# metatensor/metatrain

Hardware: AMD Instinct MI355X
Metric: atom-steps/sec (energy+forces) PET 10k-atom box (higher is better)
Workload: dtype f32; 1 GPU; PET forward + dE/dR (preprocess+features+predict+backward), 8 x 10000-atom boxes per GPU per step, default PET hypers (2.9M params), 4.5 A cutoff, 191050 edges/box; parallelism=boxes sharded over 1 rank(s), no data-path collective

## Files before the change

### metatrain_amd/csrc/model.h

```cpp
#pragma once
#include <map>
#include <set>
#include <string>
#include <vector>

#include "common.h"
#include "switches.h"

namespace pet {

constexpr int D = 128;
constexpr int DN = 256;
constexpr int DFF = 256;
constexpr int DNF = 2 * DN;
constexpr int DH = 128;
constexpr int NHEAD = 8;
constexpr int HD = D / NHEAD;
constexpr int MAX_SPECIES = 128;

struct Lin {
    const float* w = nullptr;
    const float* b = nullptr;
    float4* fwd = nullptr;
    float4* bwd = nullptr;
// ... 140 lines not shown
constexpr int MAILBOX_INTS = 64;
int read_back(const int* d_a, int na, const int* d_b, int nb, int* out, hipStream_t st);
int64_t graph_workspace_bytes(int64_t n_nodes, int64_t e0);
int graph_attention_lists(const Graph& g, hipStream_t st);
int graph_build(const Model& m, const float* pos, const float* cells, const int* centers,
                const int* neighbors, const int* shifts, const int* species, const int* sys,
                int64_t n_nodes, int64_t e0, int64_t n_systems, void* ws, int64_t ws_bytes,
                Graph& g, hipStream_t st);
int graph_check_reverse(Graph& g, hipStream_t st);
int64_t graph_from_batch_workspace_bytes(int64_t n_nodes, int64_t max_nbr);
int graph_from_batch(const int64_t* el_nodes, const int64_t* el_nbr, const float* ev, const float* ed, const uint8_t* mask,
                     const int64_t* rni, const float* cf, int64_t n_nodes, int64_t max_nbr, void* ws, int64_t ws_bytes,
                     Graph& g, hipStream_t st);
int graph_export(const Graph& g, float cutoff, int64_t* el_nodes, int64_t* el_nbr, float* ev,
                 float* ed, uint8_t* mask, int64_t* rni, float* cf, float* stats, int64_t* centers,
                 int64_t* neighbors, int64_t* slot, int64_t* shifts, hipStream_t st);
int sum_over_atoms(const Graph& g, const float* atomic, float* out, hipStream_t st);

int64_t nl_workspace_bytes(int64_t n_atoms);
int64_t nl_batch_workspace_bytes(int64_t n_atoms, int64_t n_systems);
int nl_build_batch(const float* d_pos, const float* h_cells, const int* h_pbc, const int64_t* h_first_atom, int64_t n_sys,
                   float cutoff, void* ws, int* d_pairs, float* d_vectors, int64_t capacity, int64_t* n_pairs,
                   hipStream_t st);
int nl_build(const float* d_pos, const float* h_cell, const int* h_pbc, int64_t n, float cutoff,
             void* ws, int* d_pairs, float* d_vectors, int64_t capacity, int64_t* n_pairs,
             hipStream_t st);

bool use_generic(const Model& m, const Graph& g);

int64_t gen_workspace_bytes(const Model& m, int64_t n_nodes, int64_t n_edges);
int gen_forward_layers(const Model& m, const Graph& g, void* ws, int64_t ws_bytes, int save, float* atomic,
                       float* const* node_feats, float* const* edge_feats, int n_layers, hipStream_t st);
int gen_backward_features(const Model& m, const Graph& g, void* ws, int64_t ws_bytes, const float* const* g_node,
                          const float* const* g_edge, int n_layers, float* g_geo, float* g_fc, hipStream_t st);
int gen_backward(const Model& m, const Graph& g, void* ws, int64_t ws_bytes, const float* gA, float* gpos, float* gcell,
                 hipStream_t st);
int gen_predict(const Model& m, const Graph& g, const HeadW& H, const LastW& Lw, const float* node_feat,
                const float* edge_feat, const float* fc, float* atomic, float* node_hidden, float* edge_hidden,
                hipStream_t st);
int gen_predict_backward(const Model& m, const Graph& g, const HeadW& H, const LastW& Lw, const float* node_feat,
                         const float* edge_feat, const float* fc, const float* gA, float* g_node, float* g_edge, float* g_fc,
                         hipStream_t st);
int gen_aux_outputs(const Model& m, const Graph& g, const float* node_feat, const float* edge_feat, float* feature,
                    float* last_layer, float* scratch, hipStream_t st);
int gen_backward_predict(const Model& m, const Graph& g, void* ws, int64_t ws_bytes, const float* gA, float* g_node,
                         float* g_edge, float* g_fc, hipStream_t st);
int gen_backward_geometry(const Model& m, const Graph& g, void* ws, int64_t ws_bytes, const float* g_geo, const float* g_fc,
                          float* gpos, float* gcell, hipStream_t st);
int64_t gen_train_workspace_bytes(const Model& m, int64_t n_nodes, int64_t n_edges);
int norm_rev_rows(const float* Xp, const float* Xt, const float* gamma, int ln, float eps, const float* NYp, const float* NYt,
                  float* NXp, float* NXt, int64_t R, int W, hipStream_t st);
struct HvpTaps {
    float *ngeo, *lgeo;
    float *sb, *sdb;
    float *db, *dbd;
    float *dfc, *dfcd;
    float* dv;
};
int gen_train2(const Model& m, const Graph& g, void* ws2, int64_t ws2_bytes, const float* lA, const float* nA, const float* u,
               const float* ucell, float* tangent_atomic, hipStream_t st, const float* const* seed_node = nullptr,
               const float* const* seed_edge = nullptr, int n_seed = 0, const HvpTaps* hv = nullptr);
int64_t gen_hvp_workspace_bytes(const Model& m, int64_t n_nodes, int64_t n_edges);
int gen_hvp(const Model& m, const Graph& g, void* ws, int64_t ws_bytes, const float* lA, const float* u, const float* ucell,
            float* hvp_pos, float* hvp_cell, float* tangent_atomic, hipStream_t st);
int gen_train_predict(const Model& m, const Graph& g, void* ws, int64_t ws_bytes, int layer, const HeadW& H, const LastW& Lw,
                      float* atomic, hipStream_t st);
int gen_train_predict_backward(const Model& m, const Graph& g, void* ws, int64_t ws_bytes, int layer, const HeadW& H,
                               int n_blocks, const LastW* const* Lw, const float* const* gA, float* seed_node,
                               float* seed_edge, hipStream_t st);
inline bool train_generic(const Model& m) { return m.generic() || !m.trainable(); }
inline bool train_generic_for(const Model& m, const Graph& g) { return train_generic(m) || use_generic(m, g) || g.n_edges == 0; }
bool generic_workspace(const Graph& g, const void* ws);
int backward_geometry_generic(const Model& m, const Graph& g, float* dv_scratch, const float* dgeo, const float* dfc_a,
                              const float* dfc_b, float* gpos, float* gcell, hipStream_t st);

int64_t forward_workspace_bytes(const Model& m, int64_t n_nodes, int64_t n_edges, bool train = false);
int forward(const Model& m, const Graph& g, void* ws, int64_t ws_bytes, int save, float* atomic,
            float* node_feat, float* edge_feat, hipStream_t st);
int forward_layers(const Model& m, const Graph& g, void* ws, int64_t ws_bytes, int save, float* atomic,
                   float* const* node_feats, float* const* edge_feats, int n_layers, hipStream_t st);
int backward_features_layers_abi(const Model& m, const Graph& g, void* ws, int64_t ws_bytes, const float* const* g_node,
                                 const float* const* g_edge, int n_layers, float* g_geo, float* g_fc, hipStream_t st);
int backward(const Model& m, const Graph& g, void* ws, int64_t ws_bytes, const float* grad_atomic,
             float* grad_pos, float* grad_cells, hipStream_t st);
int64_t predict_scratch_floats(int64_t n_nodes, int64_t n_edges);
int predict(const Model& m, const Graph& g, const HeadW& H, const LastW& Lw, const float* node_feat, const float* edge_feat,
            const float* fc, float* atomic, float* node_hidden, float* edge_hidden, float* scratch, hipStream_t st);
int predict_backward(const Model& m, const Graph& g, const HeadW& H, const LastW& Lw, const float* node_feat,
                     const float* edge_feat, const float* fc, const float* grad_atomic, float* g_node, float* g_edge,
                     float* g_fc, float* scratch, hipStream_t st);
int aux_outputs(const Model& m, const Graph& g, const float* node_feat, const float* edge_feat, float* feature,
                float* last_layer, float* scratch, hipStream_t st);
int backward_train(const Model& m, const Graph& g, void* ws, int64_t ws_bytes, const float* grad_atomic,
                   float* grad_pos, float* grad_cells, hipStream_t st, const float* const* seed_node = nullptr,
                   const float* const* seed_edge = nullptr, int n_seed = 0);
int train_predict(const Model& m, const Graph& g, void* ws, int64_t ws_bytes, int layer, const HeadW& H, const LastW& Lw,
                  float* atomic, hipStream_t st);
int train_predict_backward(const Model& m, const Graph& g, void* ws, int64_t ws_bytes, const std::string& target, int layer,
                           const HeadW& H, int n_blocks, const char* const* blocks, const LastW* const* Lw,
                           const float* const* gA, float* seed_node, float* seed_edge, hipStream_t st);
int llpr_features(const Model& m, const Graph& g, const char* target, const char* block, const float* const* node_feats,
                  const float* const* edge_feats, int n_layers, float* atomic, float* llf, hipStream_t st);
int llpr_rows(const float* llf, int64_t N, int F, const int* sysidx, int64_t S, const uint8_t* mask, int mean, float* rows,
              hipStream_t st);
int llpr_covariance_accumulate(const float* X, int64_t R, int F, double* C, hipStream_t st);
int llpr_covariance_finalize(double* C, int F, hipStream_t st);
int llpr_variance(const float* X, int64_t R, int F, const float* M, float alpha, float* sigma, hipStream_t st);
int llpr_ensemble(const float* X, int64_t R, int F, const float* W, int K, int P, const float* pred, float* Y, hipStream_t st);
int64_t so_workspace_bytes(const Model& m, int64_t n_nodes, int64_t n_edges);
int geometry_tangent(const Model& m, const Graph& g, const float* u, const float* ucell, float* Tgeo, float* Tfc, float* Tkb,
                     hipStream_t st);
int backward_train2(const Model& m, const Graph& g, void* ws, int64_t ws_bytes, void* ws2, int64_t ws2_bytes,
                    const float* lambda_atomic, const float* nu_atomic, const float* u, float* tangent_atomic,
                    hipStream_t st, const float* u_cell = nullptr, const float* const* seed_node = nullptr,
                    const float* const* seed_edge = nullptr, int n_seed = 0);
int backward_predict_abi(const Model& m, const Graph& g, void* ws, int64_t ws_bytes, const float* grad_atomic,
                         float* g_node, float* g_edge, float* g_fc, hipStream_t st);
int backward_features_abi(const Model& m, const Graph& g, void* ws, int64_t ws_bytes, const float* g_node,
                          const float* g_edge, float* g_geo, float* g_fc, hipStream_t st);
int geometry_backward(const Model& m, const Graph& g, const float* g_geo, const float* g_fc, float* gpos, float* gcell,
                      float* scratch, hipStream_t st);
int backward_geometry_abi(const Model& m, const Graph& g, void* ws, int64_t ws_bytes, const float* g_geo,
                          const float* g_fc, float* grad_pos, float* grad_cells, hipStream_t st);

bool use_trr();
int trr_compress(bool first, const Graph& g, const GnnLayerW& G, const float* Min, float* a0_out, float* Xout, int64_t E,
                 hipStream_t st);
int trr_compress_bwd(bool first, const float* dXe, const float* a0, const GnnLayerW& G, float* dgeo, float* dM, int64_t E,
                     float* t_da0, hipStream_t st);
int trr_head_edge(const Model& m, const float* Xin, const float* fc, float* ypred, float* yout, int64_t E, hipStream_t st);
int trr_head_edge_bwd(const Model& m, const float* Xin, const float* gA, const int* ctr, const float* fc, const float* ypred,
                      float* dfc, float* dXout, int64_t E, float* t_s1, float* t_da2, float* t_da1, float* t_s2y, hipStream_t st);
void trr_qkv(const float* X, const float* gamma, const float* beta, const Lin& qkv, float* QKV, int64_t R, hipStream_t st);
void trr_qkv_bwd(const float* dQKV, const float* X, const float* gamma, bool layer_norm, const Lin& qkv, const float* dX1,
                 float* dXin, int64_t E, int64_t R, hipStream_t st);
void trr_oproj(const float* AO, const float* X, const Lin& out, float* X1, float* OC, int64_t E, int64_t R, hipStream_t st);
void trr_oproj_bwd(const float* dX1, const float* dOC, const Lin& out, float* dAO, int64_t E, int64_t R, hipStream_t st);
void trr_emlp(const float* X1, const float* gamma, const float* beta, const Lin& win, const Lin& wout, float* VG, float* X2,
              int64_t E, hipStream_t st);
void trr_emlp_bwd(const float* dY, const float* X1, const float* VG, const float* gamma, const float* beta, const Lin& win,
                  const Lin& wout, float* dX1, int64_t E, hipStream_t st, float* t_dvg = nullptr, int ldy = 128,
                  const float* dY2 = nullptr, const int* rev2 = nullptr);
int trr_comb(bool first, const float* XF, const Graph& g, const GnnLayerW& G, const float* Min, const float* edge_emb, float* CA,
             float* LNS, float* Mout, int64_t E, hipStream_t st);
int trr_comb_bwd(const float* dM, const float* XF, const Graph& g, const GnnLayerW& G, const float* LNS, const float* CA,
                 float* dcat, int64_t E, float* t_da, hipStream_t st, bool add_dm = false);
int emlp_s(const float* X1, const float* gamma, const float* beta, const Lin& win, const Lin& wout, float* VG, float* X2,
           int64_t E, hipStream_t st);
int emlp_bwd_s(const float* dY, const float* X1, bool ln, const Lin& win_g, const Lin& wout, float* dX1, int64_t E,
               hipStream_t st, int ldy, const float* dY2, const int* rev2);
int head_edge_s(const Model& m, const float* Xin, const float* fc, float* ypred, float* yout, int64_t E, hipStream_t st);
int head_edge_bwd_s(const Model& m, const float* Xin, const float* gA, const int* ctr, const float* fc, const float* ypred,
                    float* dfc, float* dXout, int64_t E, hipStream_t st);
int compress_bwd_s(bool first, const float* dXe, const float* a0, const GnnLayerW& G, float* dgeo, float* dM, int64_t E, hipStream_t st);
int comb_s(bool first, const float* XF, const int* rev, const Lin& c0g, const Lin& c2, const float* Min, const float* edge_emb,
           const int* sp_nbr, float* CA, float* LNS, float* Mout, int64_t E, hipStream_t st);
int comb_bwd_s(const float* dM, const float* XF, const int* rev, const float* LNS, const float* CA, const Lin& c0g, const Lin& c2,
               float* dcat, int64_t E, bool add_dm, hipStream_t st);
int center_s(const Lin& cc, const float* H, float* Xc, int64_t N, hipStream_t st);
int expand_bwd_s(const Lin& ce, const float* dH1, float* dOC, int64_t N, hipStream_t st);
int center_bwd_s(const Lin& cc, const float* dC, const float* dH1, float* dHin, int64_t N, hipStream_t st);
int node_fwd_s(const AttnLayerW& A, const float* H, const float* OC, float* H1, float* VGn, float* Hn, float* tmp, int64_t N,
               hipStream_t st);
int node_bwd_s(const AttnLayerW& A, const float* dHn, const float* H1, const float* VGn, float* dH1, float* tmp, int64_t N, bool ln,
               hipStream_t st);
int ablk_fwd(const Model& m, const Graph& g, const AttnLayerW& A, const float* X, float* X1, float* OC, float scale, hipStream_t st);
int ablk_bwd(const Model& m, const Graph& g, const AttnLayerW& A, const float* X, const float* dX1, const float* dOC, float* dXin,
             float* dbias, float scale, hipStream_t st);
void ablk_prof_dump();
bool rowgemm_s(hipStream_t st, const float* X, int K, const float* cs, const void* planes, const float* bias, float* Y, int n_out,
               int64_t R, bool acc);
bool rowgemm_s_ex(hipStream_t st, const float* X, int K, const float* cs, const void* planes, const float* bias, const float* A,
                  float* Y, int n_out, int64_t R, int norm, const float* cb);
bool rowgemm_s_swiglu_bwd(hipStream_t st, const float* X, const void* planes, const float* VG, float* dVG, int hid, int64_t R);
bool rowgemm_s_norm_bwd(hipStream_t st, const float* X, int K, const void* planes, const float* xn, const float* gamma, int ln,
                        const float* dres, float* out, int64_t R);

bool attn_fwd_preload(int nt, const float* QKV, const Graph& g, float* AO, float scale, hipStream_t st);
bool attn_bwd_preload(int nt, const float* QKV, const float* dAO, const Graph& g, float* dQKV, float* dbias_h,
                      float scale, hipStream_t st);

bool attn_jvp_mfma(int nt, const float* QKV, const float* QKVd, const Graph& g, const float* Tkb, float* AOd,
                   float scale, hipStream_t st);
bool attn_rev_mfma(int nt, const float* QKV, const float* QKVd, const Graph& g, const float* Tkb, const float* LO,
                   const float* NO, float* lQKV, float* nQKV, float scale, hipStream_t st);

struct SideStream {
    hipStream_t s = nullptr;
    hipEvent_t to_side = nullptr, to_main = nullptr;
    bool enabled = false;
    hipStream_t stream(hipStream_t main) const { return enabled ? s : main; }
    void fork(hipStream_t main) const;
    void join(hipStream_t main) const;
};
const SideStream& side_stream();

struct ProfScope {
    ProfScope(const char* name, hipStream_t st, double flops, double bytes = 0.0);
    ~ProfScope();
    const char* name;
    hipStream_t st;
    double flops;
    double bytes = 0.0;
    hipEvent_t e0 = nullptr, e1 = nullptr;
};

}

struct pet_graph {
    pet::Graph g;
    float cutoff;
};
```

### metatrain_amd/csrc/pet_compress_s.hip

```cpp
#include "rows_s.h"

namespace pet {

__device__ __forceinline__ void cs_pin(float4 (&x)[16]) {
#pragma unroll
    for (int k = 0; k < 16; k++) asm volatile("" : "+v"(x[k].x), "+v"(x[k].y), "+v"(x[k].z), "+v"(x[k].w));
}
__device__ __forceinline__ void cs_piece(const W2& m, int r, unsigned dst, int wave, unsigned lane16) {
    const int tp = (r >> 3) & 1, kb = r & 7;
    ab_dma_piece((wave & 1) ? m.l : m.h, (2 * tp + (wave >> 1)) * 8 + kb, lane16, dst);
}

template <bool FIRST>
__global__ __launch_bounds__(256, 2) void k_compress_bwd_s(const float* __restrict__ dXe, const float* __restrict__ a0, W2 w2b,
                                                          W2 wcp , W2 w0cb,
                                                          float* __restrict__ dgeo, float* __restrict__ dM, int64_t E) {
    extern __shared__ __attribute__((aligned(16))) char cs_smem[];
    const RowLane L;
    const unsigned lane16 = (unsigned)L.lane * 16u;
    const int wave = __builtin_amdgcn_readfirstlane(threadIdx.x >> 6);
    int64_t row0 = ((int64_t)blockIdx.x * HS_NW + wave) * WROWS;
    const bool live = row0 < E;
    if (!live) row0 = ((E - 1) / WROWS) * WROWS;
    const int64_t row = row0 + L.r < E ? row0 + L.r : E - 1;
    const bool valid = live && row0 + L.r < E;
    char* tile = cs_smem + wave * 16384;
    const char* ring = cs_smem + HS_NW * 16384;
    const unsigned tile_u = __builtin_amdgcn_readfirstlane((unsigned)(uintptr_t)tile);
    const unsigned ring_u = __builtin_amdgcn_readfirstlane((unsigned)(uintptr_t)ring);
    constexpr int NST = FIRST ? 20 : 36;
    auto req = [&](int g) {
        g = g < NST ? g : NST - 1;
        const unsigned dst = ring_u + (unsigned)(g & (HS_NSLOT - 1)) * HS_SLOT + wave * 1024;
        if (g < 16) cs_piece(w2b, g, dst, wave, lane16);
        else if (g < 20) ab_dma_piece((wave & 1) ? wcp.l : wcp.h, 2 * (g - 16) + (wave >> 1), lane16, dst);
        else cs_piece(w0cb, g - 20, dst, wave, lane16);
    };
    dma_tile128(dXe, row0, E, tile_u, L);
    float4 d[16];
    load_rowfrag<16>(d, a0, row, D, L.h);
    cs_pin(d);
    asm volatile("s_waitcnt vmcnt(0)" ::: "memory");
    req(0);
    req(1);
    req(2);
    f16x8 xh[8], xl[8];
    f32x16 acc[4];
    float inv;
    {
        float4 x[16];
        tile128_to_frag(x, tile, L);
        float sc;
        inv = row_scale_pow2<16>(x, sc);
        hs_planes(x, xh, xl);
    }
#pragma unroll
    for (int t = 0; t < 4; t++) acc[t] = ab_zero();
    hs_gemm_r(acc, xh, xl, 0, req, ring, lane16);
    {
        const float f = inv * ABQ_INV;
#pragma unroll
        for (int t = 0; t < 4; t++)
#pragma unroll
            for (int j = 0; j < 4; j++) {
                float4& a = d[4 * t + j];
                a = make_float4(acc[t][4 * j] * f * silu_g_(a.x), acc[t][4 * j + 1] * f * silu_g_(a.y), acc[t][4 * j + 2] * f * silu_g_(a.z),
                                acc[t][4 * j + 3] * f * silu_g_(a.w));
            }
        float sc;
        inv = row_scale_pow2<16>(d, sc);
        hs_planes(d, xh, xl);
    }
    f32x16 gt = ab_zero();
#pragma unroll
    for (int r = 0; r < 4; r++) {
        const int g = 16 + r;
        HS_STAGE_SYNC();
        req(g + 3);
        const char* slot = ring + (g & (HS_NSLOT - 1)) * HS_SLOT + lane16;
#pragma unroll
        for (int j = 0; j < 2; j++) {
            const f16x8 wh = *reinterpret_cast<const f16x8*>(slot + (2 * j) * 1024);
            const f16x8 wl = *reinterpret_cast<const f16x8*>(slot + (2 * j + 1) * 1024);
            AB_MFMA3(gt, wh, wl, xh[2 * r + j], xl[2 * r + j]);
        }
    }
    if (!FIRST) {
#pragma unroll
        for (int t = 0; t < 4; t++) acc[t] = ab_zero();
        hs_gemm_r(acc, xh, xl, 20, req, ring, lane16);
    }
    const float f = inv * ABQ_INV;
    if (valid && L.h == 0) {
        float4* dg = reinterpret_cast<float4*>(dgeo + row * 4);
        const float4 old = *dg;
        *dg = make_float4(fmaf(gt[0], f, old.x), fmaf(gt[1], f, old.y), fmaf(gt[2], f, old.z), fmaf(gt[3], f, old.w));
    }
    if (!FIRST) {
        auto rows = [&](int r) { return dM + (row0 + r < E ? row0 + r : E - 1) * D; };
        float4 old[16], y[16];
        request_rows_addend<16>(old, L, rows);
#pragma unroll
        for (int t = 0; t < 4; t++)
#pragma unroll
            for (int j = 0; j < 4; j++)
                y[4 * t + j] = make_float4(acc[t][4 * j] * f, acc[t][4 * j + 1] * f, acc[t][4 * j + 2] * f, acc[t][4 * j + 3] * f);
        __builtin_amdgcn_wave_barrier();
        asm volatile("" ::: "memory");
        store_rows_lines_add<16>(y, old, reinterpret_cast<float*>(tile), L,
                                 [&](int r) { return live && row0 + r < E ? dM + (row0 + r) * D : nullptr; });
    }
}

static inline W2 cs_w2(const void* base, int tiles, int kbs) {
    const f16x8* b = reinterpret_cast<const f16x8*>(base);
    W2 w; w.h = b; w.l = b + (size_t)tiles * kbs * 64;
    return w;
}

int compress_bwd_s(bool first, const float* dXe, const float* a0, const GnnLayerW& G, float* dgeo, float* dM, int64_t E,
                   hipStream_t st) {
    PET_REQUIRE_PLANES(G.compress2.bwd2s && G.wc2s && (first || G.compress0_msg.bwd2s), "compress adjoint");
    const size_t lds = HS_NW * 16384 + HS_NSLOT * HS_SLOT;
    const int grid = (int)cdiv(E, HS_NW * WROWS);
    const W2 w2b = cs_w2(G.compress2.bwd2s, D / 32, D / 16), wcp = cs_w2(G.wc2s, 1, D / 16);
    if (first) {
        allow_big_lds(k_compress_bwd_s<true>, lds);
        k_compress_bwd_s<true><<<grid, 256, lds, st>>>(dXe, a0, w2b, wcp, W2(), dgeo, nullptr, E);
    } else {
        allow_big_lds(k_compress_bwd_s<false>, lds);
        k_compress_bwd_s<false><<<grid, 256, lds, st>>>(dXe, a0, w2b, wcp, cs_w2(G.compress0_msg.bwd2s, D / 32, D / 16), dgeo, dM, E);
    }
    return PET_OK;
}

}
```

### metatrain_amd/csrc/pet_fwd.hip

```cpp
#include <mutex>
#include <set>

#include "common.h"
#include "model.h"
#include "pet_ws.h"
#include "tile.h"

namespace pet {

constexpr int LD128 = lds_ld(128);
constexpr int LD256 = lds_ld(256);

template <int NT>
__device__ __forceinline__ void store_acc(f32x16 (&acc)[NT], float* __restrict__ G, int64_t row0,
                                          int64_t n_rows, int ld, int rb, int col0, int lane) {
    acc_foreach<NT>(acc, rb, col0, lane, [&](int r, int c, float v) {
        if (row0 + r < n_rows) G[(row0 + r) * ld + c] = v;
    });
}

__global__ void k_node_embed(const int* __restrict__ sp, const float* __restrict__ emb,
                             float* __restrict__ H, int n) {
    int64_t idx = (int64_t)blockIdx.x * blockDim.x + threadIdx.x;
    if (idx >= (int64_t)n * (DN / 4)) return;
// ... 806 lines not shown
}
__global__ void k_rows_scatter(const float* __restrict__ buf, const int* __restrict__ rows, int64_t n, float* __restrict__ X,
                               int mode) {
    const int64_t idx = (int64_t)blockIdx.x * blockDim.x + threadIdx.x;
    if (idx >= n * (D / 4)) return;
    const int64_t r = idx / (D / 4);
    const int c = (int)(idx % (D / 4));
    float4* dst = reinterpret_cast<float4*>(X + (int64_t)rows[r] * D) + c;
    if (mode == 2) { *dst = make_float4(0.f, 0.f, 0.f, 0.f); return; }
    const float4 v = reinterpret_cast<const float4*>(buf)[idx];
    if (mode == 0) *dst = v;
    else { float4 o = *dst; o.x += v.x; o.y += v.y; o.z += v.z; o.w += v.w; *dst = o; }
}
int exchange_forward(const Graph& g, float* XF, int layer, hipStream_t st) {
    if (!g.x_fn) return PET_OK;
    if (g.n_export > 0)
        k_rows_gather<<<cdiv(g.n_export * (D / 4), 256), 256, 0, st>>>(XF, g.x_export, g.n_export, g.x_export_buf);
    PET_REQUIRE(g.x_fn(g.x_user, 0, layer) == 0, PET_ERR_ARGUMENT, "the exchange callback failed (forward)");
    if (g.n_ghost > 0)
        k_rows_scatter<<<cdiv(g.n_ghost * (D / 4), 256), 256, 0, st>>>(g.x_ghost_buf, g.x_ghost, g.n_ghost, XF, 0);
    PET_HIP_CHECK(hipGetLastError());
    return PET_OK;
}
int exchange_backward(const Graph& g, float* dXF, int layer, hipStream_t st) {
    if (!g.x_fn) return PET_OK;
    if (g.n_ghost > 0) {
        k_rows_gather<<<cdiv(g.n_ghost * (D / 4), 256), 256, 0, st>>>(dXF, g.x_ghost, g.n_ghost, g.x_ghost_buf);
        k_rows_scatter<<<cdiv(g.n_ghost * (D / 4), 256), 256, 0, st>>>(nullptr, g.x_ghost, g.n_ghost, dXF, 2);
    }
    PET_REQUIRE(g.x_fn(g.x_user, 1, layer) == 0, PET_ERR_ARGUMENT, "the exchange callback failed (reverse)");
    if (g.n_export > 0)
        k_rows_scatter<<<cdiv(g.n_export * (D / 4), 256), 256, 0, st>>>(g.x_export_buf, g.x_export, g.n_export, dXF, 1);
    PET_HIP_CHECK(hipGetLastError());
    return PET_OK;
}

int64_t forward_workspace_bytes(const Model& m, int64_t n_nodes, int64_t n_edges, bool train) {
    if (m.generic() || (train && train_generic(m))) return gen_workspace_bytes(m, n_nodes, n_edges);
    Workspace w;
    carve_workspace(m, n_nodes, n_edges, nullptr, w, train);
    return (int64_t)w.bytes;
}

template <int NT>
static void launch_attn_fwd(const float* QKV, const Graph& g, float* AO, float scale, hipStream_t st) {
    int waves = (int)g.n_nodes * NHEAD;
    k_attn_fwd<NT><<<cdiv(waves, 4), 256, 0, st>>>(QKV, g.rowptr, g.fc, AO, g.n_edges, (int)g.n_nodes, scale);
}

int attn_tiles(const Graph& g) { return (g.max_nbr + 1 + 15) / 16; }
bool use_generic(const Model& m, const Graph& g) { return m.generic() || attn_tiles(g) > 8; }
bool generic_workspace(const Graph& g, const void* ws) {
    const Graph::FwdRecord* r = g.fwd_record(ws);
    return r && r->generic;
}
static Graph::FwdRecord& note_workspace(const Graph& g, const void* ws, bool generic) {
    Graph::FwdRecord& r = g.fwd_record_new(ws);
    r.generic = generic;
    return r;
}

double g_sum_t2(const Graph& g) {
    if (g.n_nodes == 0) return 0.0;
    const double t = (double)g.n_edges / (double)g.n_nodes + 1.0;
    return (double)g.n_nodes * t * t;
}

static inline WX wx_fwd(const Lin& L) {
    WX w;
    w.f = L.fwd;
    if (L.fwd2) {
        const size_t n8 = (size_t)(L.n_out / 32) * (L.k_in / 16) * 64;
        w.h = reinterpret_cast<const f16x8_t*>(L.fwd2);
        w.l = w.h + n8;
    }
    return w;
}

int forward(const Model& m, const Graph& g, void* ws, int64_t ws_bytes, int save, float* atomic,
            float* node_feat, float* edge_feat, hipStream_t st) {
    PET_REQUIRE(!m.residual() || (!node_feat && !edge_feat), PET_ERR_ARGUMENT,
                "residual featuriser: one feature pair per GNN layer, use pet_forward_layers");
    return forward_layers(m, g, ws, ws_bytes, save, atomic, &node_feat, &edge_feat, 1, st);
}

int forward_layers(const Model& m, const Graph& g, void* ws, int64_t ws_bytes, int save, float* atomic,
                   float* const* node_feats, float* const* edge_feats, int n_layers, hipStream_t st) {
    const bool gen = use_generic(m, g) || (save == 2 && train_generic_for(m, g));
    PET_REQUIRE(!(gen && g.x_fn), PET_ERR_UNSUPPORTED, "the per-layer exchange is built for the tuned path (default model size)");
    Graph::FwdRecord& fwd_rec = note_workspace(g, ws, gen);
    fwd_rec.save = save;
    if (gen) return gen_forward_layers(m, g, ws, ws_bytes, save, atomic, node_feats, edge_feats, n_layers, st);
    if (int rcl = graph_attention_lists(g, st)) return rcl;
    Workspace w;
    carve_workspace(m, g.n_nodes, g.n_edges, ws, w, save == 2);
    PET_REQUIRE((int64_t)w.bytes <= ws_bytes, PET_ERR_ARGUMENT, "forward workspace too small");
    const bool post = m.post_ln(), res = m.residual();
    PET_REQUIRE(res ? (n_layers == m.h.num_gnn_layers || (n_layers == 1 && !node_feats[0] && !edge_feats[0])) : n_layers == 1,
                PET_ERR_ARGUMENT, "expected one feature pair per readout layer (" + std::to_string(m.num_readout_layers()) + ")");
    PET_REQUIRE(!(atomic && res), PET_ERR_UNSUPPORTED,
                "the fused head reads one readout layer; with the residual featuriser use pet_forward_layers and "
                "pet_predict per readout layer");
    PET_REQUIRE(save != 2 || m.trainable(), PET_ERR_UNSUPPORTED,
                "training is built for transformer_type=PreLN, featurizer_type=feedforward only");
    const int64_t N = g.n_nodes, E = g.n_edges, R = E + N;
    if (N == 0) return PET_OK;
    const int nt = attn_tiles(g);
    const float scale = 1.0f / (sqrtf((float)HD) * m.h.attention_temperature);
    const int gE = cdiv(E, BM), gN = cdiv(N, BM), gR = cdiv(R, BM);
    const size_t lds1 = BM * LD128 * 4, lds2 = 2 * BM * LD128 * 4;
    const size_t lds_c = lds2 + BM * 20 + BM * 8;
    const double fE = (double)E, fN = (double)N, fR = (double)R;
    const StagePlan& plan = fwd_rec.plan = plan_forward(m, g, save);
    const double attn_flops = 4.0 * D * g_sum_t2(g);
    const int L = m.h.num_gnn_layers, AL = m.h.num_attention_layers;

    allow_big_lds(k_center, BM * LD256 * 4 + BM * 8);
    allow_big_lds(k_node, (BM * LD256 + BM * LD128) * 4 + BM * 8);
    allow_big_lds(k_head<256>, (BM * LD256 + BM * LD128) * 4 + BM * 8);
    SideStream ss = side_stream();
    ss.enabled = plan.side;
    const hipStream_t s2 = ss.stream(st);
    bool side_busy = false;
    auto launch_center = [&](int gi, int a) -> int {
        const AttnLayerW& A = m.gnn[gi].attn[a];
        AttnBufs& Ab = w.gnn[gi].attn[a];
        if (a == 0 && res && gi > 0)
            k_node_embed<<<cdiv(N * (DN / 4), 256), 256, 0, s2>>>(g.sp, m.node_embs[gi], w.gnn[gi].Hin, (int)N);
        ProfScope ps("center", s2, fN * 2.0 * DN * D);
        if (plan.gnn[gi].layers[a].center == Center::Ring) return center_s(A.cc, Ab.H, Ab.X + E * D, N, s2);
        k_center<<<gN, NTHREADS, BM * LD256 * 4 + BM * 8, s2>>>(Ab.H, wx_fwd(A.cc), A.cc.b, Ab.X + E * D, N);
        return PET_OK;
    };
    k_node_embed<<<cdiv(N * (DN / 4), 256), 256, 0, st>>>(g.sp, m.node_emb, w.H0, (int)N);
    const bool conditioned = m.h.system_conditioning != 0;
    if (conditioned) {
        PET_REQUIRE(g.cond_charge && g.n_cond_systems >= 1 && g.n_cond_systems <= N, PET_ERR_ARGUMENT,
                    "system_conditioning: call pet_graph_set_conditioning (charge, spin multiplicity, system indices) first");
        k_system_cond<<<(int)g.n_cond_systems, DN, 0, st>>>(g.cond_charge, g.cond_spin, m.cond_qe, m.cond_se, m.cond_w0,
                                                             m.cond_b0, m.cond_w2, m.cond_b2, w.cond, m.h.max_charge,
                                                             m.h.max_spin_multiplicity);
    }
    ss.fork(st);
    PET_TRY(launch_center(0, 0));
    side_busy = true;
    bool node_cnt_zeroed = false;
    for (int gi = 0; gi < L; gi++) {
        const GnnLayerW& G = m.gnn[gi];
        GnnBufs& B = w.gnn[gi];
        const GnnPlan& P = plan.gnn[gi];
        const float* Min = gi == 0 ? nullptr : w.gnn[gi - 1].Mout;
        if (E > 0) {
            ProfScope ps("compress", st, fE * 2.0 * (D * D * (gi == 0 ? 3 : 4) + 4 * D));
            if (P.compress == Rows::Pipelined)
                PET_TRY(trr_compress(gi == 0, g, G, Min, save == 0 ? nullptr : B.a0, B.attn[0].X, E, st));
            else if (gi == 0)
                k_compress<true><<<gE, NTHREADS, lds1 + BM * 20 + BM * 8, st>>>(g.geo, g.sp_nbr, G.wc, G.tbl, nullptr, WX(),
                                                                        wx_fwd(G.compress2), G.compress2.b, B.a0,
                                                                        B.attn[0].X, E);
            else
                k_compress<false><<<gE, NTHREADS, lds_c, st>>>(g.geo, g.sp_nbr, G.wc, G.tbl, Min,
                                                               wx_fwd(G.compress0_msg), wx_fwd(G.compress2), G.compress2.b,
                                                               B.a0, B.attn[0].X, E);
        }
        for (int a = 0; a < AL; a++) {
            const AttnLayerW& A = G.attn[a];
            AttnBufs& Ab = B.attn[a];
            const LayerPlan& Q = P.layers[a];
            float* Xnext = (a + 1 < AL) ? B.attn[a + 1].X : B.XF;
            if (side_busy) {
                ss.join(st);
                side_busy = false;
            }
            const bool trr_l = Q.attn == Attn::Pipelined;
            if (Q.attn == Attn::Fused) {
                ProfScope ps("attn_blk", st, fR * 2.0 * D * 4 * D + attn_flops, fR * 4.0 * 2 * D);
                PET_TRY(ablk_fwd(m, g, A, Ab.X, Ab.X1, Ab.OC, scale, st));
            } else {
            {
                ProfScope ps("qkv", st, fR * 2.0 * D * 3 * D, fR * 4.0 * (D + 3 * D));
                if (trr_l) trr_qkv(Ab.X, A.g_attn, m.layer_norm() ? A.b_attn : nullptr, A.qkv, Ab.QKV, R, st);
                else if (post) k_qkv<false><<<gR, NTHREADS, lds1, st>>>(Ab.X, nullptr, nullptr, A.qkv.fwd, A.qkv.b, Ab.QKV, R);
                else k_qkv<true><<<gR, NTHREADS, lds1, st>>>(Ab.X, A.g_attn, A.b_attn, A.qkv.fwd, A.qkv.b, Ab.QKV, R);
            }
            {
                ProfScope ps("attn_fwd", st, attn_flops, fR * 4.0 * (3 * D + D));
                if (!(plan.attn_preload && attn_fwd_preload(nt, Ab.QKV, g, Ab.AO, scale, st))) switch (nt) {
                    case 1: launch_attn_fwd<1>(Ab.QKV, g, Ab.AO, scale, st); break;
                    case 2: launch_attn_fwd<2>(Ab.QKV, g, Ab.AO, scale, st); break;
                    case 3: launch_attn_fwd<3>(Ab.QKV, g, Ab.AO, scale, st); break;
                    case 4: launch_attn_fwd<4>(Ab.QKV, g, Ab.AO, scale, st); break;
                    case 5: case 6: launch_attn_fwd<6>(Ab.QKV, g, Ab.AO, scale, st); break;
                    default: launch_attn_fwd<8>(Ab.QKV, g, Ab.AO, scale, st); break;
                }
            }
            {
                ProfScope ps("oproj", st, fR * 2.0 * D * D, fR * 4.0 * 3 * D);
                if (trr_l) trr_oproj(Ab.AO, Ab.X, A.out, Ab.X1, Ab.OC, E, R, st);
                else if (post) k_oproj<true><<<gR, NTHREADS, lds1, st>>>(Ab.AO, Ab.X, A.out.fwd, A.out.b, Ab.X1, nullptr, E, R);
                else k_oproj<false><<<gR, NTHREADS, lds1, st>>>(Ab.AO, Ab.X, A.out.fwd, A.out.b, Ab.X1, Ab.OC, E, R);
            }
            }
            if (post) {
                ProfScope ps("emlp", st, fR * 2.0 * (D * 2 * DFF + DFF * D));
                k_rownorm<<<gR, NTHREADS, lds1, st>>>(Ab.X1, A.g_attn, A.b_attn, w.T1, w.T1 + E * D, E, R);
                k_emlp<false><<<gR, NTHREADS, lds2, st>>>(w.T1, nullptr, nullptr, A.mlp_in.fwd, A.mlp_in.b, A.mlp_out.fwd,
                                                           A.mlp_out.b, Ab.VG, Ab.S2, R);
                k_rownorm<<<gR, NTHREADS, lds1, st>>>(Ab.S2, A.g_mlp, A.b_mlp, Xnext, Ab.OC, E, R);
            }
            ss.fork(st);
            const bool has_next = a + 1 < AL || gi + 1 < L;
            const AttnLayerW* An = !has_next ? nullptr : a + 1 < AL ? &G.attn[a + 1] : &m.gnn[gi + 1].attn[0];
            AttnBufs* Abn = !has_next ? nullptr : a + 1 < AL ? &B.attn[a + 1] : &w.gnn[gi + 1].attn[0];
            const bool center_done = has_next && (a + 1 < AL ? P.layers[a + 1] : plan.gnn[gi + 1].layers[0]).center == Center::ByNode;
            {
                ProfScope ps("node", s2, fN * 2.0 * (D * DN + DN * 2 * DNF + DNF * DN));
                WX wcn;
                const float* bcn = nullptr;
                float* xcn = nullptr;
                if (center_done) {
                    PET_REQUIRE(Abn->H == Ab.Hn, PET_ERR_ARGUMENT, "node update: the next layer does not start from this layer's node features");
                    wcn = wx_fwd(An->cc); bcn = An->cc.b; xcn = Abn->X + E * D;
                }
                const WX wci = wx_fwd(A.cmlp_in), wce_ = wx_fwd(A.ce), wco = wx_fwd(A.cmlp_out);
                const int nr = Q.node == Node::Rows64 ? 64 : 32;
                const size_t lds_n2 = (size_t)nr * LD256 * 4 + (size_t)2 * nr * plane_ld(256) * 2 + nr * 8;
                switch (Q.node) {
                case Node::Ring:
                    PET_TRY(node_fwd_s(A, Ab.H, Ab.OC, Ab.H1, Ab.VGn, Ab.Hn, w.dQKV, N, s2));
                    break;
                case Node::Split: {
                    const int nt32 = cdiv(N, 32);
                    const size_t p_floats = (size_t)(DNF / 128) * nt32 * 32 * DN;
                    int* cnt = reinterpret_cast<int*>(w.dQKV + p_floats);
                    if (!node_cnt_zeroed) PET_HIP_CHECK(hipMemsetAsync(cnt, 0, nt32 * sizeof(int), s2));
                    node_cnt_zeroed = true;
                    allow_big_lds(k_node2<1, true>, lds_n2);
                    k_node2<1, true><<<dim3(nt32, DNF / 128), NTHREADS, lds_n2, s2>>>(
                        Ab.H, Ab.OC, wce_, A.ce.b, A.g_center, A.b_center, wci, A.cmlp_in.b, wco, A.cmlp_out.b, Ab.H1, Ab.VGn,
                        Ab.Hn, N, wcn, bcn, xcn, w.dQKV, cnt);
                    break;
                }
                case Node::Rows32:
                    allow_big_lds(k_node2<1>, lds_n2);
                    k_node2<1><<<cdiv(N, 32), NTHREADS, lds_n2, s2>>>(Ab.H, Ab.OC, wce_, A.ce.b, A.g_center, A.b_center, wci,
                                                                     A.cmlp_in.b, wco, A.cmlp_out.b, Ab.H1, Ab.VGn, Ab.Hn, N,
                                                                     wcn, bcn, xcn, nullptr, nullptr);
                    break;
                case Node::Rows64:
                    allow_big_lds(k_node2w, lds_n2);
                    k_node2w<<<gN, NTHREADS, lds_n2, s2>>>(Ab.H, Ab.OC, wce_, A.ce.b, A.g_center, A.b_center, wci,
                                                           A.cmlp_in.b, wco, A.cmlp_out.b, Ab.H1, Ab.VGn, Ab.Hn, N, wcn, bcn, xcn);
                    break;
                case Node::LdsTile:
                    k_node<<<gN, NTHREADS, (BM * LD256 + BM * LD128) * 4 + BM * 8, s2>>>(
                        Ab.H, Ab.OC, wce_, A.ce.b, A.g_center, A.b_center, wci, A.cmlp_in.b, wco, A.cmlp_out.b, Ab.H1, Ab.VGn,
                        Ab.Hn, N);
                    break;
                }
            }
            if (a + 1 == AL && conditioned)
                k_add_cond<<<cdiv(N * (DN / 4), 256), 256, 0, s2>>>(Ab.Hn, w.cond, g.sys, g.cond_sys, (int)N);
            if (has_next && !center_done) PET_TRY(a + 1 < AL ? launch_center(gi, a + 1) : launch_center(gi + 1, 0));
            side_busy = true;
            if (E > 0 && !post) {
                ProfScope ps("emlp", st, fE * 2.0 * (D * 2 * DFF + DFF * D), fE * 4.0 * (2 * D + (Q.emlp_saved ? 2 * DFF : 0)));
                float* vg = Q.emlp_saved ? Ab.VG : nullptr;
                const float* beta = m.layer_norm() ? A.b_mlp : nullptr;
                switch (Q.emlp) {
                case Rows::Ring: PET_TRY(emlp_s(Ab.X1, A.g_mlp, beta, A.mlp_in, A.mlp_out, vg, Xnext, E, st)); break;
                case Rows::Pipelined: trr_emlp(Ab.X1, A.g_mlp, beta, A.mlp_in, A.mlp_out, vg, Xnext, E, st); break;
                case Rows::LdsTile:
                    k_emlp<true><<<gE, NTHREADS, lds2, st>>>(Ab.X1, A.g_mlp, A.b_mlp, A.mlp_in.fwd, A.mlp_in.b, A.mlp_out.fwd,
                                                             A.mlp_out.b, Ab.VG, Xnext, E);
                    break;
                }
            }
        }
        if (g.x_fn) {
            PET_REQUIRE(m.plain() && save != 2, PET_ERR_UNSUPPORTED,
                        "the per-layer exchange is built for PreLN + feedforward models, inference and forces");
            int rc = exchange_forward(g, B.XF, gi, st);
            if (rc) return rc;
        }
        if (E > 0 && res) {
            if (gi + 1 < L) {
                ProfScope ps("comb", st, 0.0, fE * 4.0 * 3 * D);
                k_resmix<<<cdiv(E * (D / 4), 256), 256, 0, st>>>(Min, m.edge_emb, g.sp_nbr, B.XF, g.rev, B.Mout, E);
            }
        } else if (E > 0) {
            ProfScope ps("comb", st, fE * 2.0 * (2 * D * 2 * D + 2 * D * D), fE * 4.0 * (3 * D + 2 * D + D));
            if (P.comb == Rows::Ring)
                PET_TRY(comb_s(gi == 0, B.XF, g.rev, G.comb0_g, G.comb2, Min, m.edge_emb, g.sp_nbr, B.CA, B.LNS, B.Mout, E, st));
            else
                PET_TRY(trr_comb(gi == 0, B.XF, g, G, Min, m.edge_emb, B.CA, B.LNS, B.Mout, E, st));
        }
    }
    const GnnBufs& last = w.gnn.back();
    if (atomic) {
        PET_REQUIRE(m.has_fused_head, PET_ERR_ARGUMENT,
                    "pet_forward with d_atomic needs the fused single-property target (keys 'node_heads.@...'); use "
                    "pet_predict for other heads");
    }
    if (atomic) {
        ProfScope ps("head_node", s2, fN * 2.0 * (DN * DH + DH * DH + DH));
        k_head<256><<<gN, NTHREADS, (BM * LD256 + BM * LD128) * 4 + BM * 8, s2>>>(
            last.Hout, wx_fwd(m.nh0), m.nh0.b, wx_fwd(m.nh2), m.nh2.b, m.nll_w, m.nll_b, nullptr, nullptr, w.ynode, N);
// ... 112 lines not shown
```

### metatrain_amd/csrc/pet_plan.h

```cpp
#pragma once
#include <stdint.h>

#include <vector>

namespace pet {

constexpr int64_t EMLP_S_MIN_ROWS = 28672;
constexpr int ABLK_MIN_TILES = 3840;
constexpr int64_t NODE_ROWS32_MAX_ATOMS = 16384;
constexpr int NODE_SPLIT_MAX_TILES = 128;
constexpr int64_t CENTER_BWD_DEEP_MAX_ATOMS = 4096;

enum class Rows : uint8_t { LdsTile, Pipelined, Ring };
enum class Attn : uint8_t { LdsTile, Pipelined, Fused };
enum class Node : uint8_t { LdsTile, Rows64, Rows32, Split, Ring };
enum class Center : uint8_t { LdsTile, Ring, ByNode };

struct LayerPlan {
    Attn attn = Attn::LdsTile;
    Rows emlp = Rows::LdsTile;
    bool emlp_saved = true;
    Node node = Node::LdsTile;
    Center center = Center::LdsTile;
    Center expand = Center::LdsTile;
};
struct GnnPlan {
    Rows compress = Rows::LdsTile;
    Rows comb = Rows::Pipelined;
    std::vector<LayerPlan> layers;
};
struct StagePlan {
    std::vector<GnnPlan> gnn;
    Rows head_edge = Rows::LdsTile;
    bool side = false;
    bool side_heads = false;
    bool dxf_fused = false;
    bool center_bwd_deep = false;
    bool attn_preload = false;
    int dbias_stride = 1;
    bool unsaved_attn() const;
};

struct Model;
struct Graph;
struct FwdRecord;
StagePlan plan_forward(const Model& m, const Graph& g, int save);
int plan_backward(const Model& m, const Graph& g, const FwdRecord* rec, bool train, StagePlan& plan);

}
```

### metatrain_amd/csrc/pet_plan.hip

```cpp
#include "pet_plan.h"

#include "common.h"
#include "model.h"

namespace pet {

static bool ring_serves(int64_t rows) { return switches().emlp_s && rows >= switches().emlp_s_rows; }
static bool ring_center_serves(int64_t N) {
    return ring_serves((int64_t)1 << 40) && (N >= NODE_ROWS32_MAX_ATOMS || switches().emlp_s_rows < EMLP_S_MIN_ROWS);
}
static bool emlp_recompute_on(const Lin& win, const Lin& wout, int64_t E) {
    return ring_serves(E) && win.fwd2s && wout.fwd2s && wout.bwd2s;
}
static bool ablk_serves(const Graph& g) {
    if (g.bucket_start[5] > g.bucket_start[4]) return false;
    if (!g.tiles_planned) return false;
    if (switches().attn_fused & 4) return true;
    return g.n_tiles1 >= ABLK_MIN_TILES && (int64_t)g.n_tiles2 * 20 <= g.n_nodes;
}
static bool ablk_bwd_on(const Graph& g) { return (switches().attn_fused & 2) && ablk_serves(g); }
static Node node_planes_form(int64_t N, size_t cap) {
    if (switches().node_planes != 2 && N > NODE_ROWS32_MAX_ATOMS) return Node::Rows64;
    const int nt32 = cdiv(N, 32);
    const size_t p_floats = (size_t)(DNF / 128) * nt32 * 32 * DN;
    return switches().node_split && nt32 <= NODE_SPLIT_MAX_TILES && p_floats + nt32 <= cap ? Node::Split : Node::Rows32;
}

bool StagePlan::unsaved_attn() const {
    for (const GnnPlan& G : gnn)
        for (const LayerPlan& A : G.layers)
            if (A.attn == Attn::Fused) return true;
    return false;
}

StagePlan plan_forward(const Model& m, const Graph& g, int save) {
    const Switches& sw = switches();
    const int64_t N = g.n_nodes, E = g.n_edges, R = E + N;
    const int L = m.h.num_gnn_layers, AL = m.h.num_attention_layers;
    StagePlan p;
    p.gnn.assign(L, GnnPlan{Rows::LdsTile, Rows::Pipelined, std::vector<LayerPlan>(AL)});
    const bool trr = use_trr();
    const bool trr_l = trr && m.plain_layers();
    const bool conditioned = m.h.system_conditioning != 0, res = m.residual();
    p.attn_preload = trr;
    p.side = p.side_heads = side_stream().enabled && !m.post_ln();
    const bool fused_ok = trr_l && save != 2 && E > 0 && (save == 0 || ablk_bwd_on(g)) && (sw.attn_fused & 1) && ablk_serves(g);
    const bool center_ring = save != 2 && ring_center_serves(N);
    for (int gi = 0; gi < L; gi++) {
        const GnnLayerW& G = m.gnn[gi];
        GnnPlan& P = p.gnn[gi];
        if (trr && (sw.trr_compress & 1) && G.compress2.fwd2 && (gi == 0 || G.compress0_msg.fwd2) && E > 0) P.compress = Rows::Pipelined;
        if (G.comb0.fwd2 && G.comb2.fwd2 && ring_serves(E) && G.comb0_g.fwd2s && G.comb2.fwd2s) P.comb = Rows::Ring;
        for (int a = 0; a < AL; a++) {
            const AttnLayerW& A = G.attn[a];
            LayerPlan& Q = P.layers[a];
            Q.attn = fused_ok && A.qkv.fwd2s && A.out.fwd2s ? Attn::Fused : trr_l ? Attn::Pipelined : Attn::LdsTile;
            if (trr_l) {
                Q.emlp = ring_serves(E) && A.mlp_in.fwd2s && A.mlp_out.fwd2s ? Rows::Ring : Rows::Pipelined;
                Q.emlp_saved = save != 0 && !(save == 1 && emlp_recompute_on(A.mlp_in, A.mlp_out, E));
            } else {
                Q.emlp_saved = save != 0;
            }
            if (sw.node_planes && (size_t)N * DNF <= (size_t)R * 3 * D && ring_serves(N) && A.ce.fwd2s && A.cmlp_in.fwd2s &&
                A.cmlp_out.fwd2s && N > 0)
                Q.node = Node::Ring;
            else if (sw.node_planes && A.cmlp_in.fwd2 && A.ce.fwd2 && A.cmlp_out.fwd2)
                Q.node = node_planes_form(N, (size_t)R * 3 * D);
            if (a + 1 < AL || gi + 1 < L) {
                const AttnLayerW& An = a + 1 < AL ? G.attn[a + 1] : m.gnn[gi + 1].attn[0];
                LayerPlan& Qn = a + 1 < AL ? P.layers[a + 1] : p.gnn[gi + 1].layers[0];
                const bool by_node = (Q.node == Node::Split || Q.node == Node::Rows32) && sw.center_fused &&
                                     !(a + 1 == AL && (conditioned || res)) && An.cc.fwd2;
                Qn.center = by_node ? Center::ByNode : center_ring && An.cc.fwd2s ? Center::Ring : Center::LdsTile;
            }
        }
    }
    if (L > 0 && AL > 0 && center_ring && m.gnn[0].attn[0].cc.fwd2s) p.gnn[0].layers[0].center = Center::Ring;
    if (trr && (sw.trr_compress & 2) && m.eh0.fwd2 && m.eh2.fwd2)
        p.head_edge = ring_serves(E) && m.eh0.fwd2s && m.eh2.fwd2s ? Rows::Ring : Rows::Pipelined;
    return p;
}

int plan_backward(const Model& m, const Graph& g, const FwdRecord* rec, bool tr, StagePlan& p) {
    const Switches& sw = switches();
    const int64_t N = g.n_nodes, E = g.n_edges, R = E + N;
    const int L = m.h.num_gnn_layers, AL = m.h.num_attention_layers;
    p = StagePlan();
    p.gnn.assign(L, GnnPlan{Rows::LdsTile, Rows::Pipelined, std::vector<LayerPlan>(AL)});
    const bool trr = use_trr();
    const bool trr_l = trr && m.plain_layers();
    const bool res = m.residual();
    const bool enabled = side_stream().enabled;
    p.attn_preload = trr;
    p.side_heads = enabled && !tr;
    p.side = enabled && !(tr || m.post_ln() || res);
    if (trr && (sw.trr_compress & 2) && m.eh0.fwd2 && m.eh2.fwd2 && m.eh0.bwd2 && m.eh2.bwd2)
        p.head_edge = !tr && ring_serves(E) && m.eh0.fwd2s && m.eh2.fwd2s && m.eh0.bwd2s && m.eh2.bwd2s ? Rows::Ring : Rows::Pipelined;
    if (L == 0 || AL == 0) return PET_OK;
    const bool fused_attn = trr_l && !tr && ablk_bwd_on(g) && m.gnn[0].attn[0].qkv.bwd2s;
    PET_REQUIRE(!rec || rec->save != 0, PET_ERR_ARGUMENT,
                "the last forward into this workspace ran with save_for_backward = 0: nothing was kept for an adjoint");
    PET_REQUIRE(!(rec && rec->plan.unsaved_attn()) || fused_attn, PET_ERR_ARGUMENT,
                "the forward of this workspace ran the fused attention block (Q, K, V not saved) but the adjoint is "
                "configured for the three-kernel form: pet_config_set changed between forward and backward");
    const bool rec_layers = rec && (int)rec->plan.gnn.size() == L;
    p.dxf_fused = trr_l && !tr && !res && !g.x_fn && AL >= 1 && sw.dxf_fused;
    p.dbias_stride = fused_attn ? NHEAD : 1;
    p.center_bwd_deep = N <= CENTER_BWD_DEEP_MAX_ATOMS;
    const bool center_ring = !tr && ring_center_serves(N);
    for (int gi = 0; gi < L; gi++) {
        const GnnLayerW& G = m.gnn[gi];
        GnnPlan& P = p.gnn[gi];
        if (!tr && ring_serves(E) && G.comb0_g.bwd2s && G.comb2.bwd2s && G.comb0_g.b) P.comb = Rows::Ring;
        if (trr && (sw.trr_compress & 1) && G.compress2.bwd2 && G.wc2 && (gi == 0 || G.compress0_msg.bwd2) && E > 0)
            P.compress = !tr && ring_serves(E) && G.compress2.bwd2s && G.wc2s && (gi == 0 || G.compress0_msg.bwd2s) ? Rows::Ring : Rows::Pipelined;
        for (int a = 0; a < AL; a++) {
            const AttnLayerW& A = G.attn[a];
            LayerPlan& Q = P.layers[a];
            if (!tr && sw.node_planes && (size_t)N * 3 * DNF <= (size_t)R * D && ring_serves(N) && A.cmlp_in.bwd2s &&
                A.cmlp_out.bwd2s && N > 0)
                Q.node = Node::Ring;
            else if (!tr && sw.node_planes && A.cmlp_out.bwd2 && A.cmlp_in.bwd2)
                Q.node = node_planes_form(N, (size_t)R * D);
            Q.expand = Q.node == Node::Split || Q.node == Node::Rows32 ? Center::ByNode : center_ring && A.ce.bwd2s ? Center::Ring : Center::LdsTile;
            Q.center = center_ring && A.cc.bwd2s ? Center::Ring : Center::LdsTile;
            const bool recompute = rec ? rec_layers && !rec->plan.gnn[gi].layers[a].emlp_saved
                                       : !tr && trr_l && emlp_recompute_on(A.mlp_in, A.mlp_out, E);
            Q.emlp_saved = !recompute;
            Q.emlp = recompute ? Rows::Ring : trr_l ? Rows::Pipelined : Rows::LdsTile;
            PET_REQUIRE(!recompute || (!tr && trr_l && sw.emlp_s && A.mlp_in_g.fwd2s && A.mlp_in_g.bwd2s && A.mlp_out.bwd2s),
                        PET_ERR_ARGUMENT, "the forward of this workspace did not save the edge MLP's pre-activations "
                        "and the recomputing adjoint is switched off: pet_config_set changed between forward and backward");
            Q.attn = fused_attn ? Attn::Fused : trr_l ? Attn::Pipelined : Attn::LdsTile;
        }
    }
    return PET_OK;
}

}
```

### metatrain_amd/csrc/switches.h

```cpp
#pragma once
#include <stdint.h>

#include "pet_plan.h"

namespace pet {

struct Switches {
    int side_stream = -1;
    int trr = -1;
    int attn_fused = 3;
    int emlp_s = 1;
    int64_t emlp_s_rows = EMLP_S_MIN_ROWS;
    int trr_compress = 3;
    int node_planes = 1;
    int so_trr = 1;
    int soap_ps_mfma = 1;
    int node_split = 1;
    int center_fused = 1;
    int sorted_shortcut = 1;
    int dxf_fused = 1;
    int train_bf16 = 0;
    int wgrad_bf16 = 1;
    int so_f16x3 = 1;
    int soap_mfma = 1;
    int soap_packed = 1;
    int soap_sorted = 1;
    int soap_pair = 1;
};

const Switches& switches();

}
```

Baseline: 1.886 million atom-steps/s.

## Add ring-pipelined compress forward kernel with LDS-staged species table

Adds a new forward compress kernel that computes the geometry projection plus species-table lookup from LDS-staged weights, then runs the message GEMM and output GEMM through the split-f16 ring-DMA pipeline already used in the backward pass. It is enabled by default for large edge counts by setting bit 4 in the compress switch and selecting the Ring plan when species count, save mode and plane weights allow. The intent is to replace the pipelined compress path with the higher-throughput ring kernel. It relies on split f16 planes, which may introduce small precision differences, and it is limited to at most 27 species.

```diff
diff --git a/metatrain_amd/csrc/model.h b/metatrain_amd/csrc/model.h
--- a/metatrain_amd/csrc/model.h
+++ b/metatrain_amd/csrc/model.h
@@ -316,6 +316,7 @@
 int head_edge_s(const Model& m, const float* Xin, const float* fc, float* ypred, float* yout, int64_t E, hipStream_t st);
 int head_edge_bwd_s(const Model& m, const float* Xin, const float* gA, const int* ctr, const float* fc, const float* ypred,
                     float* dfc, float* dXout, int64_t E, hipStream_t st);
+int compress_s(bool first, const Graph& g, const GnnLayerW& G, int ns, const float* Min, float* a0_out, float* Xout, int64_t E, hipStream_t st);
 int compress_bwd_s(bool first, const float* dXe, const float* a0, const GnnLayerW& G, float* dgeo, float* dM, int64_t E, hipStream_t st);
 int comb_s(bool first, const float* XF, const int* rev, const Lin& c0g, const Lin& c2, const float* Min, const float* edge_emb,
            const int* sp_nbr, float* CA, float* LNS, float* Mout, int64_t E, hipStream_t st);
diff --git a/metatrain_amd/csrc/pet_compress_s.hip b/metatrain_amd/csrc/pet_compress_s.hip
--- a/metatrain_amd/csrc/pet_compress_s.hip
+++ b/metatrain_amd/csrc/pet_compress_s.hip
@@ -112,10 +112,150 @@
     }
 }
 
+constexpr int CS_TBL_LD = 132;
+static_assert(4 * (D * 4 + COMPRESS_S_MAX_SPECIES * CS_TBL_LD) <= HS_NSLOT * HS_SLOT, "Wc and the Tbl rows fit the ring area");
+
+template <bool FIRST>
+__global__ __launch_bounds__(256, 2) void k_compress_s(const float4* __restrict__ geo, const int* __restrict__ sp_nbr,
+                                                      const float* __restrict__ wc , const float* __restrict__ tbl ,
+                                                      int ns, const float* __restrict__ Min, W2 w0c, W2 w2, const float* __restrict__ b2,
+                                                      float* __restrict__ a0_out, float* __restrict__ Xout, int64_t E) {
+    extern __shared__ __attribute__((aligned(16))) char cs_smem[];
+    const RowLane L;
+    const unsigned lane16 = (unsigned)L.lane * 16u;
+    const int wave = __builtin_amdgcn_readfirstlane(threadIdx.x >> 6);
+    int64_t row0 = ((int64_t)blockIdx.x * HS_NW + wave) * WROWS;
+    const bool live = row0 < E;
+    if (!live) row0 = ((E - 1) / WROWS) * WROWS;
+    const int64_t row = row0 + L.r < E ? row0 + L.r : E - 1;
+    char* tile = cs_smem + wave * 16384;
+    char* ring = cs_smem + HS_NW * 16384;
+    const unsigned tile_u = __builtin_amdgcn_readfirstlane((unsigned)(uintptr_t)tile);
+    const unsigned ring_u = __builtin_amdgcn_readfirstlane((unsigned)(uintptr_t)ring);
+    constexpr int NST = FIRST ? 16 : 32;
+    auto req = [&](int g) {
+        g = g < NST ? g : NST - 1;
+        const unsigned dst = ring_u + (unsigned)(g & (HS_NSLOT - 1)) * HS_SLOT + wave * 1024;
+        if (!FIRST && g < 16) cs_piece(w0c, g, dst, wave, lane16);
+        else cs_piece(w2, g & 15, dst, wave, lane16);
+    };
+    if (!FIRST) dma_tile128(Min, row0, E, tile_u, L);
+    float4 a[16];
+    {
+        const float4 g = geo[row];
+        const int sp = sp_nbr[row];
+        float4* stg = reinterpret_cast<float4*>(ring);
+        const int n4 = D + ns * (D / 4);
+        for (int i = threadIdx.x; i < n4; i += 256) {
+            const int t = i - D;
+            stg[i < D ? i : D + (t >> 5) * (CS_TBL_LD / 4) + (t & 31)] =
+                i < D ? reinterpret_cast<const float4*>(wc)[i] : reinterpret_cast<const float4*>(tbl)[t];
+        }
+        asm volatile("s_waitcnt vmcnt(0) lgkmcnt(0)" ::: "memory");
+        __syncthreads();
+        const float4* ws = stg + 4 * L.h;
+        const float4* ts = stg + D + sp * (CS_TBL_LD / 4) + L.h;
+#pragma unroll
+        for (int kg = 0; kg < 16; kg++) {
+            const float4 t = ts[2 * kg];
+            const float4 w0 = ws[8 * kg], w1 = ws[8 * kg + 1], w2v = ws[8 * kg + 2], w3 = ws[8 * kg + 3];
+            a[kg].x = fmaf(g.w, w0.w, fmaf(g.z, w0.z, fmaf(g.y, w0.y, g.x * w0.x))) + t.x;
+            a[kg].y = fmaf(g.w, w1.w, fmaf(g.z, w1.z, fmaf(g.y, w1.y, g.x * w1.x))) + t.y;
+            a[kg].z = fmaf(g.w, w2v.w, fmaf(g.z, w2v.z, fmaf(g.y, w2v.y, g.x * w2v.x))) + t.z;
+            a[kg].w = fmaf(g.w, w3.w, fmaf(g.z, w3.z, fmaf(g.y, w3.y, g.x * w3.x))) + t.w;
+        }
+        cs_pin(a);
+        asm volatile("s_waitcnt lgkmcnt(0)" ::: "memory");
+        __syncthreads();
+    }
+    req(0);
+    req(1);
+    req(2);
+    f16x8 xh[8], xl[8];
+    f32x16 acc[4];
+    float inv;
+    if (!FIRST) {
+        {
+            float4 x[16];
+            tile128_to_frag(x, tile, L);
+            float sc;
+            inv = row_scale_pow2<16>(x, sc);
+            hs_planes(x, xh, xl);
+        }
+#pragma unroll
+        for (int t = 0; t < 4; t++) acc[t] = ab_zero();
+        hs_gemm_r(acc, xh, xl, 0, req, ring, lane16);
+        const float f = inv * ABQ_INV;
+#pragma unroll
+        for (int t = 0; t < 4; t++)
+#pragma unroll
+            for (int j = 0; j < 4; j++) {
+                float4& v = a[4 * t + j];
+                v = make_float4(fmaf(acc[t][4 * j], f, v.x), fmaf(acc[t][4 * j + 1], f, v.y), fmaf(acc[t][4 * j + 2], f, v.z),
+                                fmaf(acc[t][4 * j + 3], f, v.w));
+            }
+    }
+    float4* const a0p = reinterpret_cast<float4*>(tile);
+    if (a0_out) {
+        __builtin_amdgcn_wave_barrier();
+        asm volatile("" ::: "memory");
+#pragma unroll
+        for (int kg = 0; kg < 16; kg++) a0p[kg * 64 + L.lane] = a[kg];
+    }
+    {
+#pragma unroll
+        for (int kg = 0; kg < 16; kg++) a[kg] = make_float4(silu_(a[kg].x), silu_(a[kg].y), silu_(a[kg].z), silu_(a[kg].w));
+        float sc;
+        inv = row_scale_pow2<16>(a, sc);
+        hs_planes(a, xh, xl);
+    }
+#pragma unroll
+    for (int t = 0; t < 4; t++) acc[t] = ab_zero();
+    hs_gemm_r(acc, xh, xl, FIRST ? 0 : 16, req, ring, lane16);
+    if (a0_out) {
+#pragma unroll
+        for (int kg = 0; kg < 16; kg++) a[kg] = a0p[kg * 64 + L.lane];
+        __builtin_amdgcn_wave_barrier();
+        asm volatile("" ::: "memory");
+        store_rows_lines<16>(a, reinterpret_cast<float*>(tile), L,
+                             [&](int r) { return live && row0 + r < E ? a0_out + (row0 + r) * D : nullptr; });
+    }
+    {
+        const float f = inv * ABQ_INV;
+#pragma unroll
+        for (int t = 0; t < 4; t++)
+#pragma unroll
+            for (int j = 0; j < 4; j++)
+                a[4 * t + j] = make_float4(fmaf(acc[t][4 * j], f, hs_vec_s(b2, t, j, 0, L.h)), fmaf(acc[t][4 * j + 1], f, hs_vec_s(b2, t, j, 1, L.h)),
+                                           fmaf(acc[t][4 * j + 2], f, hs_vec_s(b2, t, j, 2, L.h)), fmaf(acc[t][4 * j + 3], f, hs_vec_s(b2, t, j, 3, L.h)));
+    }
+    __builtin_amdgcn_wave_barrier();
+    asm volatile("" ::: "memory");
+    store_rows_lines<16>(a, reinterpret_cast<float*>(tile), L, [&](int r) { return live && row0 + r < E ? Xout + (row0 + r) * D : nullptr; });
+}
+
 static inline W2 cs_w2(const void* base, int tiles, int kbs) {
     const f16x8* b = reinterpret_cast<const f16x8*>(base);
     W2 w; w.h = b; w.l = b + (size_t)tiles * kbs * 64;
     return w;
+}
+
+int compress_s(bool first, const Graph& g, const GnnLayerW& G, int ns, const float* Min, float* a0_out, float* Xout, int64_t E,
+               hipStream_t st) {
+    PET_REQUIRE_PLANES(G.compress2.fwd2s && (first || G.compress0_msg.fwd2s), "compress stage");
+    PET_REQUIRE(ns >= 1 && ns <= COMPRESS_S_MAX_SPECIES, PET_ERR_ARGUMENT, "compress stage: the species table does not fit the ring area");
+    const size_t lds = HS_NW * 16384 + HS_NSLOT * HS_SLOT;
+    const int grid = (int)cdiv(E, HS_NW * WROWS);
+    const W2 w2 = cs_w2(G.compress2.fwd2s, D / 32, D / 16);
+    if (first) {
+        allow_big_lds(k_compress_s<true>, lds);
+        k_compress_s<true><<<grid, 256, lds, st>>>(g.geo, g.sp_nbr, G.wc, G.tbl, ns, nullptr, W2(), w2, G.compress2.b, a0_out, Xout, E);
+    } else {
+        allow_big_lds(k_compress_s<false>, lds);
+        k_compress_s<false><<<grid, 256, lds, st>>>(g.geo, g.sp_nbr, G.wc, G.tbl, ns, Min, cs_w2(G.compress0_msg.fwd2s, D / 32, D / 16), w2,
+                                                     G.compress2.b, a0_out, Xout, E);
+    }
+    return PET_OK;
 }
 
 int compress_bwd_s(bool first, const float* dXe, const float* a0, const GnnLayerW& G, float* dgeo, float* dM, int64_t E,
diff --git a/metatrain_amd/csrc/pet_fwd.hip b/metatrain_amd/csrc/pet_fwd.hip
--- a/metatrain_amd/csrc/pet_fwd.hip
+++ b/metatrain_amd/csrc/pet_fwd.hip
@@ -982,7 +982,10 @@
         const float* Min = gi == 0 ? nullptr : w.gnn[gi - 1].Mout;
         if (E > 0) {
             ProfScope ps("compress", st, fE * 2.0 * (D * D * (gi == 0 ? 3 : 4) + 4 * D));
-            if (P.compress == Rows::Pipelined)
+            if (P.compress == Rows::Ring) {
+                ProfScope pr("compress_s", st, 0.0);
+                PET_TRY(compress_s(gi == 0, g, G, m.h.n_species, Min, save == 0 ? nullptr : B.a0, B.attn[0].X, E, st));
+            } else if (P.compress == Rows::Pipelined)
                 PET_TRY(trr_compress(gi == 0, g, G, Min, save == 0 ? nullptr : B.a0, B.attn[0].X, E, st));
             else if (gi == 0)
                 k_compress<true><<<gE, NTHREADS, lds1 + BM * 20 + BM * 8, st>>>(g.geo, g.sp_nbr, G.wc, G.tbl, nullptr, WX(),
diff --git a/metatrain_amd/csrc/pet_plan.h b/metatrain_amd/csrc/pet_plan.h
--- a/metatrain_amd/csrc/pet_plan.h
+++ b/metatrain_amd/csrc/pet_plan.h
@@ -6,6 +6,7 @@
 namespace pet {
 
 constexpr int64_t EMLP_S_MIN_ROWS = 28672;
+constexpr int COMPRESS_S_MAX_SPECIES = 27;
 constexpr int ABLK_MIN_TILES = 3840;
 constexpr int64_t NODE_ROWS32_MAX_ATOMS = 16384;
 constexpr int NODE_SPLIT_MAX_TILES = 128;
diff --git a/metatrain_amd/csrc/pet_plan.hip b/metatrain_amd/csrc/pet_plan.hip
--- a/metatrain_amd/csrc/pet_plan.hip
+++ b/metatrain_amd/csrc/pet_plan.hip
@@ -8,6 +8,11 @@
 static bool ring_serves(int64_t rows) { return switches().emlp_s && rows >= switches().emlp_s_rows; }
 static bool ring_center_serves(int64_t N) {
     return ring_serves((int64_t)1 << 40) && (N >= NODE_ROWS32_MAX_ATOMS || switches().emlp_s_rows < EMLP_S_MIN_ROWS);
+}
+static bool compress_ring_serves(const Model& m, int64_t E, int save) {
+    const Switches& sw = switches();
+    return sw.emlp_s && save != 2 && m.plain_layers() && m.h.n_species <= COMPRESS_S_MAX_SPECIES &&
+           ((sw.trr_compress & 8) || ((sw.trr_compress & 4) && E >= EMLP_S_MIN_ROWS));
 }
 static bool emlp_recompute_on(const Lin& win, const Lin& wout, int64_t E) {
     return ring_serves(E) && win.fwd2s && wout.fwd2s && wout.bwd2s;
@@ -49,7 +54,8 @@
     for (int gi = 0; gi < L; gi++) {
         const GnnLayerW& G = m.gnn[gi];
         GnnPlan& P = p.gnn[gi];
-        if (trr && (sw.trr_compress & 1) && G.compress2.fwd2 && (gi == 0 || G.compress0_msg.fwd2) && E > 0) P.compress = Rows::Pipelined;
+        if (trr && (sw.trr_compress & 1) && G.compress2.fwd2 && (gi == 0 || G.compress0_msg.fwd2) && E > 0)
+            P.compress = compress_ring_serves(m, E, save) && G.compress2.fwd2s && (gi == 0 || G.compress0_msg.fwd2s) ? Rows::Ring : Rows::Pipelined;
         if (G.comb0.fwd2 && G.comb2.fwd2 && ring_serves(E) && G.comb0_g.fwd2s && G.comb2.fwd2s) P.comb = Rows::Ring;
         for (int a = 0; a < AL; a++) {
             const AttnLayerW& A = G.attn[a];
diff --git a/metatrain_amd/csrc/switches.h b/metatrain_amd/csrc/switches.h
--- a/metatrain_amd/csrc/switches.h
+++ b/metatrain_amd/csrc/switches.h
@@ -11,7 +11,7 @@
     int attn_fused = 3;
     int emlp_s = 1;
     int64_t emlp_s_rows = EMLP_S_MIN_ROWS;
-    int trr_compress = 3;
+    int trr_compress = 7;
     int node_planes = 1;
     int so_trr = 1;
     int soap_ps_mfma = 1;
```

Result: no change. 1.900 million atom-steps/s, median of 6 (+0.8%).
